# ai-forever/Kandinsky-2

Hardware: NVIDIA H100
Metric: unet_denoising_steps_per_sec (higher is better)
Workload: dtype f16

## Files before the change

kandinsky-2_b200/csrc/k2_api.cu:

```cuda
#include <stdio.h>
#include <stdlib.h>
#include <string.h>

#include <algorithm>
#include <atomic>
#include <mutex>

#include "../../include/k2b200.h"
#include "k2_internal.h"

namespace k2 {

static thread_local std::string g_err;
static std::atomic<long long> g_launches{0};
static int g_force_bn = 0;
static int g_force_split = 0;
static int g_pdl = 0;


void set_error(const std::string& msg) { g_err = msg; }
int fail(const std::string& msg) {
  g_err = msg;
  return -1;
}
void count_launch(int n) { g_launches.fetch_add(n, std::memory_order_relaxed); }

bool pdl_enabled() { return g_pdl != 0; }
static int g_conv_epi_sets = 1;
static int g_gn_bps = 0;
int gn_apply_blocks_per_sm() { return g_gn_bps; }
static int g_attn_half = 1;
// ... 90 lines not shown
    }
  }
  const int k = (!single_image_only && best_tiles[1] * 100 <= best_tiles[0] * 85) ? 1 : 0;
  TN = bn[k];
  TW = bw[k];
  TH = bh[k];
}


struct ConvPlan {
  int TN, TH, TW, tiles_w, tiles_h, tiles_n, m_tiles;
  int m_tiles_phase;
  int BN, splits;
  int fuse_stats, row_groups;
  int es;
};

static void plan_conv(int NB, int H, int W, bool any9, int kchunks, int Cout, int out_mode, bool has_workspace,
                      long long workspace_bytes, bool want_gn, ConvPlan& pl, const int* cfg = nullptr, bool up2 = false,
                      bool w_batched = false) {
  const int g_force_bn = (cfg && cfg[0]) ? cfg[0] : k2::g_force_bn;
  const int g_force_split = (cfg && cfg[2]) ? cfg[2] : k2::g_force_split;
  pl.es = (cfg && cfg[3]) ? cfg[3] : k2::g_conv_epi_sets;
  choose_tile(NB, H, W, pl.TN, pl.TH, pl.TW, w_batched);
  pl.tiles_w = (W + pl.TW - 1) / pl.TW;
  pl.tiles_h = (H + pl.TH - 1) / pl.TH;
  pl.tiles_n = (NB + pl.TN - 1) / pl.TN;
  pl.m_tiles = pl.tiles_w * pl.tiles_h * pl.tiles_n;
  pl.m_tiles_phase = pl.m_tiles;

// ... 34 lines not shown
        if (g_force_split > 0 && sp != g_force_split) continue;
        if (!split_ok(sp)) continue;
        const long long c = model(bn, sp);
        if (best < 0 || c < best) {
          best = c;
          best_bn = bn;
          best_sp = sp;
        }
      }
    }
    BN = best_bn;
    splits = best_sp;
  }
  pl.BN = BN;
  pl.splits = splits;

  pl.fuse_stats = 0;
  pl.row_groups = 0;
  if (want_gn && out_mode == 0 && Cout % 8 == 0) {
    if (splits == 1 && BN >= 64 && Cout % 64 == 0 && (pl.TN == 1 || pl.TH * pl.TW == 16)) {
      pl.fuse_stats = 1;
      pl.row_groups = ((pl.TN == 1) ? pl.m_tiles : NB * pl.tiles_h * pl.tiles_w) * (up2 ? 4 : 1);
    } else if (splits > 1 && (static_cast<long long>(H) * W) % 16 == 0) {
      pl.fuse_stats = 2;
      pl.row_groups = static_cast<int>(M_total / 16);
    }
  }
}

static void plan_to_info(const ConvPlan& pl, int* info) {
  if (!info) return;
  info[0] = pl.BN; info[1] = 0;
  info[2] = pl.splits; info[3] = pl.m_tiles; info[4] = pl.TN;
  info[5] = pl.fuse_stats; info[6] = pl.row_groups;
}

}

using namespace k2;

extern "C" {

const char* k2_last_error(void) { return g_err.c_str(); }
int k2_version(void) { return 100; }
long long k2_launch_count(void) { return g_launches.load(); }
void k2_reset_launch_count(void) { g_launches.store(0); }
int k2_set_tuning(int key, int value) {
  if (key == 0) {
    g_force_bn = value;
    return 0;
  }
  if (key == 1) {
    g_force_split = value;
    return 0;
  }
  if (key == 2) {
    if (value == 2) return fail("k2_set_tuning: no CTA-pair conv kernel on sm_90");
    return 0;
  }
  if (key == 4) {
    g_pdl = value;
    return 0;
  }
  if (key == 10) {
    g_conv_epi_sets = (value == 2) ? 2 : 1;
    return 0;
  }
  if (key == 11) {
    g_gn_bps = value;
    return 0;
  }
  if (key == 9) {
// ... 11 lines not shown
  return k2_conv_gemm_cfg(srcs, nsrc, NB, H, W, w_packed, w_rows, Ktot, ldw, Cout, bias, residual, ldr, out, ldo, out_mode,
                          workspace, workspace_bytes, gn_partial, info, nullptr, 0, stream);
}

int k2_conv_gemm_cfg(const K2ConvSrc* srcs, int nsrc, int NB, int H, int W, const void* w_packed, int w_rows,
                     int Ktot, int ldw, int Cout, const float* bias, const void* residual, int ldr, void* out, int ldo,
                     int out_mode, void* workspace, long long workspace_bytes, float* gn_partial, int* info,
                     const int* cfg, long long w_batch_stride, k2_stream_t stream) {
  K2_REQUIRE(w_batch_stride >= 0 && w_batch_stride % 8 == 0, "conv_gemm_cfg: w_batch_stride must be a multiple of 8 elements");
  const bool w_batched = w_batch_stride > 0;
  if (cfg) {
    K2_REQUIRE(cfg[0] == 0 || cfg[0] == 16 || cfg[0] == 64 || cfg[0] == 128 || cfg[0] == 192 || cfg[0] == 256,
               "conv_gemm_cfg: N tile must be 0, 16, 64, 128, 192 or 256");
    K2_REQUIRE(cfg[1] >= 0 && cfg[1] <= 2 && cfg[2] >= 0 && cfg[2] <= 8 && cfg[3] >= 0 && cfg[3] <= 2,
               "conv_gemm_cfg: pair mode in 0..2, splits in 0..8, epilogue sets in 0..2");
    K2_REQUIRE(cfg[1] != 2, "conv_gemm_cfg: no CTA-pair conv kernel on sm_90");
  }
  K2_REQUIRE(nsrc >= 1 && nsrc <= 3, "conv_gemm: 1..3 sources");
  K2_REQUIRE(NB > 0 && H > 0 && W > 0 && Cout > 0, "conv_gemm: bad geometry");
  K2_REQUIRE(w_rows >= Cout, "conv_gemm: w_rows < Cout");
  K2_REQUIRE(Ktot % 64 == 0, "conv_gemm: Ktot must be a multiple of 64");
  if (ldw == 0) ldw = Ktot;
  K2_REQUIRE(ldw >= Ktot && ldw % 8 == 0 && (reinterpret_cast<uintptr_t>(w_packed) & 15) == 0,
             "conv_gemm: weight row stride / alignment");
  ConvGemmParams p;
  memset(&p, 0, sizeof p);
  p.NB = NB;
  p.H = H;
  p.W = W;
  bool any9 = false;
  int kchunks = 0;
// ... 13 lines not shown
    K2_REQUIRE(src.C > 0 && src.C % 8 == 0 && src.ld % 8 == 0 && src.ld >= src.C, "conv_gemm: bad source C/ld");
    K2_REQUIRE((reinterpret_cast<uintptr_t>(src.ptr) & 15) == 0, "conv_gemm: source not 16B aligned");
    any9 = any9 || src.taps == 9;
    p.seg_taps[s] = src.taps;
    p.seg_kchunks[s] = (src.C + 63) / 64;
    kchunks += src.taps * p.seg_kchunks[s];
  }
  K2_REQUIRE(kchunks * 64 * (up2 ? 4 : 1) == Ktot,
             "conv_gemm: Ktot does not match the sources (taps * ceil(C/64)*64 summed; x4 phases for a taps == 4 source)");
  p.num_k_chunks = kchunks;

  ConvPlan pl;
  plan_conv(NB, H, W, any9 || up2, kchunks, Cout, out_mode, workspace != nullptr, workspace_bytes, gn_partial != nullptr, pl,
            cfg, up2, w_batched);
  K2_REQUIRE(!w_batched || (!up2 && pl.TN == 1), "conv_gemm_cfg: batched weights need single-image tiles");
  p.w_batched = w_batched ? 1 : 0;
  plan_to_info(pl, info);
  p.TN = pl.TN;
  p.TH = pl.TH;
  p.TW = pl.TW;
  p.tiles_w = pl.tiles_w;
  p.tiles_h = pl.tiles_h;
  p.tiles_n = pl.tiles_n;
  p.m_tiles = up2 ? 4 * pl.m_tiles_phase : pl.m_tiles;
  p.m_tiles_phase = pl.m_tiles_phase;
  p.up2 = up2 ? 1 : 0;
  p.a_box_bytes = static_cast<uint32_t>(p.TN * p.TH * p.TW * 128);
  for (int s = 0; s < nsrc; ++s) {
    const K2ConvSrc& src = srcs[s];
    uint64_t dims[4] = {static_cast<uint64_t>(src.C), static_cast<uint64_t>(W), static_cast<uint64_t>(H),
// ... 2 lines not shown
                       static_cast<uint64_t>(src.ld) * 2 * W * H};
    uint32_t box[4] = {64, static_cast<uint32_t>(p.TW), static_cast<uint32_t>(p.TH), static_cast<uint32_t>(p.TN)};
    if (encode_tmap_f16(&p.tmA[s], src.ptr, 4, dims, str, box)) return -1;
  }
  const int BN = pl.BN, splits = pl.splits, fuse_stats = pl.fuse_stats;
  p.splits = splits;
  p.k_per_split = (kchunks + splits - 1) / splits;
  p.M_total = static_cast<long long>(NB) * H * W * (up2 ? 4 : 1);
  p.ws = reinterpret_cast<float*>(workspace);
  p.n_tiles = (Cout + BN - 1) / BN;
  p.Cout = Cout;
  {
    uint64_t dims[3] = {static_cast<uint64_t>(Ktot), static_cast<uint64_t>(w_rows), static_cast<uint64_t>(w_batched ? NB : 1)};
    uint64_t str[2] = {static_cast<uint64_t>(ldw) * 2,
                       (w_batched ? static_cast<uint64_t>(w_batch_stride) : static_cast<uint64_t>(ldw) * w_rows) * 2};
    uint32_t box[3] = {64, static_cast<uint32_t>(BN), 1};
    if (encode_tmap_f16(&p.tmB, w_packed, 3, dims, str, box)) return -1;
  }
  p.bias = bias;
  p.residual = reinterpret_cast<const __half*>(residual);
  p.ldr = ldr;
  p.out = out;
  p.ldo = ldo;
  p.out_mode = (splits > 1) ? 2 : out_mode;
  p.gn_part = (fuse_stats == 1) ? reinterpret_cast<float2*>(gn_partial) : nullptr;
  p.gn_mode = (fuse_stats == 1) ? (p.TN == 1 ? 1 : 2) : 0;
  if (out_mode == 0) {
    K2_REQUIRE(ldo % 8 == 0 && (reinterpret_cast<uintptr_t>(out) & 15) == 0, "conv_gemm: out alignment");
    if (residual)
      K2_REQUIRE(ldr % 8 == 0 && (reinterpret_cast<uintptr_t>(residual) & 15) == 0, "conv_gemm: residual alignment");
  }
  int rc = launch_conv_gemm(p, BN, pl.es, static_cast<cudaStream_t>(stream));
  if (rc == 0) g_launches.fetch_add(1, std::memory_order_relaxed);
  if (rc == 0 && splits > 1) {
    rc = launch_splitk_finalize(p.ws, splits, p.M_total, Cout, bias, p.residual, ldr, reinterpret_cast<__half*>(out), ldo,
                                fuse_stats == 2 ? reinterpret_cast<float2*>(gn_partial) : nullptr,
                                static_cast<cudaStream_t>(stream));
    if (rc == 0) g_launches.fetch_add(1, std::memory_order_relaxed);
  }
  return rc;
}

int k2_conv_plan(int NB, int H, int W, int taps, int Ktot, int Cout, int out_mode, long long workspace_bytes,
                 int want_gn_partial, int* info) {
  K2_REQUIRE(NB > 0 && H > 0 && W > 0 && Cout > 0 && info, "conv_plan: bad arguments");
  K2_REQUIRE(Ktot > 0 && Ktot % 64 == 0, "conv_plan: Ktot must be a positive multiple of 64");
  ConvPlan pl;
// ... 7 lines not shown
```

kandinsky-2_b200/csrc/k2_common.cuh:

```cuda
#pragma once
#include <cuda.h>
#include <cuda_fp16.h>
#include <cuda_runtime.h>
#include <stdint.h>
#include <stdio.h>

namespace k2 {

__device__ __forceinline__ uint32_t smem_u32(const void* p) {
  return static_cast<uint32_t>(__cvta_generic_to_shared(p));
}

__device__ __forceinline__ uint32_t lane_id() { return threadIdx.x & 31; }

__device__ __forceinline__ bool elect_one() {
  uint32_t pred = 0;
  asm volatile(
      "{\n"
      ".reg .b32 rx;\n"
      ".reg .pred px;\n"
      "elect.sync rx|px, 0xffffffff;\n"
      "selp.b32 %0, 1, 0, px;\n"
      "}\n"
      : "=r"(pred));
// ... 1 lines not shown
}

__device__ __forceinline__ void mbar_init(uint64_t* bar, uint32_t count) {
  asm volatile("mbarrier.init.shared::cta.b64 [%0], %1;" ::"r"(smem_u32(bar)), "r"(count));
}
__device__ __forceinline__ void fence_barrier_init() {
  asm volatile("fence.mbarrier_init.release.cluster;" ::: "memory");
}
__device__ __forceinline__ void mbar_arrive_expect_tx(uint64_t* bar, uint32_t bytes) {
  asm volatile("mbarrier.arrive.expect_tx.shared::cta.b64 _, [%0], %1;" ::"r"(smem_u32(bar)),
               "r"(bytes)
               : "memory");
}
__device__ __forceinline__ void mbar_arrive(uint64_t* bar) {
  asm volatile("mbarrier.arrive.shared::cta.b64 _, [%0];" ::"r"(smem_u32(bar)) : "memory");
}
__device__ __forceinline__ bool mbar_try_wait(uint64_t* bar, uint32_t parity) {
  uint32_t ok;
  asm volatile(
      "{\n"
      ".reg .pred p;\n"
      "mbarrier.try_wait.parity.shared::cta.b64 p, [%1], %2;\n"
      "selp.b32 %0, 1, 0, p;\n"
      "}\n"
      : "=r"(ok)
      : "r"(smem_u32(bar)), "r"(parity)
      : "memory");
  return ok != 0;
}
__device__ __forceinline__ void mbar_wait(uint64_t* bar, uint32_t parity) {
// ... 27 lines not shown
                                            int c1) {
  asm volatile(
      "cp.async.bulk.tensor.2d.shared::cluster.global.mbarrier::complete_tx::bytes [%0], [%1, {%3, "
      "%4}], [%2];"
      ::"r"(smem_u32(dst)),
      "l"(reinterpret_cast<uint64_t>(tm)), "r"(smem_u32(bar)), "r"(c0), "r"(c1)
      : "memory");
}
__device__ __forceinline__ void tma_load_3d(void* dst, const CUtensorMap* tm, uint64_t* bar, int c0,
                                            int c1, int c2) {
  asm volatile(
      "cp.async.bulk.tensor.3d.shared::cluster.global.mbarrier::complete_tx::bytes [%0], [%1, {%3, "
      "%4, %5}], [%2];"
      ::"r"(smem_u32(dst)),
      "l"(reinterpret_cast<uint64_t>(tm)), "r"(smem_u32(bar)), "r"(c0), "r"(c1), "r"(c2)
      : "memory");
}
__device__ __forceinline__ void tma_load_4d(void* dst, const CUtensorMap* tm, uint64_t* bar, int c0,
                                            int c1, int c2, int c3) {
  asm volatile(
      "cp.async.bulk.tensor.4d.shared::cluster.global.mbarrier::complete_tx::bytes [%0], [%1, {%3, "
      "%4, %5, %6}], [%2];"
      ::"r"(smem_u32(dst)),
      "l"(reinterpret_cast<uint64_t>(tm)), "r"(smem_u32(bar)), "r"(c0), "r"(c1), "r"(c2), "r"(c3)
      : "memory");
}

__device__ __forceinline__ uint64_t make_wgmma_desc(uint32_t smem_addr) {
  uint64_t d = 0;
  d |= static_cast<uint64_t>((smem_addr & 0x3FFFF) >> 4);
// ... 159 lines not shown
```

kandinsky-2_b200/csrc/k2_conv_gemm.cu:

```cuda
#include <stdio.h>

#include "k2_common.cuh"
#include "k2_internal.h"

namespace k2 {

namespace {

constexpr int BM = 128;
constexpr int BK = 64;
constexpr int A_STAGE_BYTES = BM * BK * 2;
constexpr int ACC_PAD = 4;

constexpr int EPI_STAGE_FLOATS = 32 * 33;
constexpr int EPI_BYTES = 4 * EPI_STAGE_FLOATS * 4 + 4 * 256 * 4;
constexpr int SMEM_LIMIT = 227 * 1024;

template <int BN, int ES>
struct Cfg {
  static constexpr int B_STAGE_BYTES = BN * BK * 2;
  static constexpr int STAGE_BYTES = A_STAGE_BYTES + B_STAGE_BYTES;
  static constexpr int BNC = (BN < 64) ? BN : (ES == 2 ? 128 : 64);
  static_assert(ES == 1 || BN % 128 == 0, "two epilogue sets need N tiles of 128 or 256");
  static constexpr int ACC_BYTES = BM * (BNC + ACC_PAD) * 4;
  static constexpr int BAR_BYTES = 256;
  static constexpr int FIXED = ACC_BYTES + ES * EPI_BYTES + BAR_BYTES + 1024;
  static constexpr int STAGES = (SMEM_LIMIT - FIXED) / STAGE_BYTES > 6 ? 6 : (SMEM_LIMIT - FIXED) / STAGE_BYTES;
  static constexpr int SMEM_BYTES = STAGES * STAGE_BYTES + FIXED;
  static_assert(STAGES >= 2, "conv_gemm: shared memory does not hold two pipeline stages");
};

__device__ __forceinline__ void decode_m_tile(const ConvGemmParams& p, int m_idx, int& n0, int& y0,
                                              int& x0, int& phase) {
  phase = 0;
  if (p.up2) {
    phase = m_idx / p.m_tiles_phase;
    m_idx -= phase * p.m_tiles_phase;
  }
  int tw_i = m_idx % p.tiles_w;
  int t = m_idx / p.tiles_w;
  int th_i = t % p.tiles_h;
  int tn_i = t / p.tiles_h;
  x0 = tw_i * p.TW;
  y0 = th_i * p.TH;
  n0 = tn_i * p.TN;
}

template <int N>
__device__ __forceinline__ void acc_ld(const float* src, uint32_t (&r)[N]) {
#pragma unroll
  for (int v = 0; v < N / 4; ++v) {
    const float4 t = *reinterpret_cast<const float4*>(src + 4 * v);
    r[4 * v] = __float_as_uint(t.x);
    r[4 * v + 1] = __float_as_uint(t.y);
    r[4 * v + 2] = __float_as_uint(t.z);
// ... 283 lines not shown
__global__ void __launch_bounds__(384, 1) conv_gemm_kernel(const __grid_constant__ ConvGemmParams p) {
  using C = Cfg<BN, ES>;
  constexpr int BNC = C::BNC;
  constexpr int NA = BN / 2;
  extern __shared__ uint8_t smem_raw[];
  uint8_t* smem = reinterpret_cast<uint8_t*>((reinterpret_cast<uintptr_t>(smem_raw) + 1023) &
                                             ~static_cast<uintptr_t>(1023));
  float* acc_smem = reinterpret_cast<float*>(smem + C::STAGES * C::STAGE_BYTES);
  float* stat_smem = reinterpret_cast<float*>(smem + C::STAGES * C::STAGE_BYTES + C::ACC_BYTES);
  uint64_t* full_bar = reinterpret_cast<uint64_t*>(smem + C::STAGES * C::STAGE_BYTES + C::ACC_BYTES + ES * EPI_BYTES);
  uint64_t* empty_bar = full_bar + C::STAGES;

  const int warp_idx = threadIdx.x >> 5;
  const int lane = threadIdx.x & 31;
  const int wg = warp_idx >> 2;

  if (threadIdx.x == 0) {
    tma_prefetch_desc(&p.tmB);
    for (int s = 0; s < 3; ++s)
      if (p.seg_taps[s]) tma_prefetch_desc(&p.tmA[s]);
    for (int i = 0; i < C::STAGES; ++i) {
      mbar_init(&full_bar[i], 1);
      mbar_init(&empty_bar[i], 8);
    }
    fence_barrier_init();
  }
  __syncthreads();
  pdl_wait();
  pdl_launch();

  const int total_tiles = p.m_tiles * p.n_tiles * p.splits;

  if (wg == 0) {
    setmaxnreg_dec<40>();
    if (warp_idx == 0 && elect_one()) {
      int stage = 0;
      uint32_t ring_phase = 0;
      const uint32_t tx_bytes = p.a_box_bytes + C::B_STAGE_BYTES;
      for (int tile = blockIdx.x; tile < total_tiles; tile += gridDim.x) {
        const int m_idx = tile % p.m_tiles;
        const int n_idx = (tile / p.m_tiles) % p.n_tiles;
        const int split = tile / (p.m_tiles * p.n_tiles);
        int n0, y0, x0, phase;
        decode_m_tile(p, m_idx, n0, y0, x0, phase);
        const int kb = phase * p.num_k_chunks;
        const int k0 = split * p.k_per_split;
        const int k1 = min(p.num_k_chunks, k0 + p.k_per_split);
        int s = 0, rem = k0;
        while (rem >= p.seg_taps[s] * p.seg_kchunks[s]) {
          rem -= p.seg_taps[s] * p.seg_kchunks[s];
          ++s;
        }
        int tap = rem / p.seg_kchunks[s];
        int c = rem - tap * p.seg_kchunks[s];
        for (int kc = k0; kc < k1; ++kc) {
          const int taps = p.seg_taps[s];
          const int dy = (taps == 9) ? (tap / 3 - 1) : (taps == 4 ? (tap >> 1) + (phase >> 1) - 1 : 0);
          const int dx = (taps == 9) ? (tap % 3 - 1) : (taps == 4 ? (tap & 1) + (phase & 1) - 1 : 0);
          mbar_wait_lean(&empty_bar[stage], ring_phase ^ 1);
          uint8_t* sA = smem + stage * C::STAGE_BYTES;
          uint8_t* sB = sA + A_STAGE_BYTES;
          mbar_arrive_expect_tx(&full_bar[stage], tx_bytes);
          tma_load_4d(sA, &p.tmA[s], &full_bar[stage], c * BK, x0 + dx, y0 + dy, n0);
          tma_load_3d(sB, &p.tmB, &full_bar[stage], (kb + kc) * BK, n_idx * BN, p.w_batched ? n0 : 0);
          if (++stage == C::STAGES) {
            stage = 0;
            ring_phase ^= 1;
          }
          if (++c == p.seg_kchunks[s]) {
            c = 0;
            if (++tap == taps) {
              tap = 0;
              ++s;
            }
          }
        }
      }
    }
  } else {
    setmaxnreg_inc<232>();
    const int g = wg - 1;
    const int w = warp_idx & 3;
    int stage = 0;
    uint32_t phase = 0;
    for (int tile = blockIdx.x; tile < total_tiles; tile += gridDim.x) {
      const int m_idx = tile % p.m_tiles;
      const int n_idx = (tile / p.m_tiles) % p.n_tiles;
      const int split = tile / (p.m_tiles * p.n_tiles);
      const int nk = min(p.num_k_chunks, (split + 1) * p.k_per_split) - split * p.k_per_split;
      float acc[NA];
#pragma unroll
      for (int i = 0; i < NA; ++i) acc[i] = 0.f;
      int prev_stage = -1;
      for (int kc = 0; kc < nk; ++kc) {
        mbar_wait_lean(&full_bar[stage], phase);
        const uint32_t a_addr = smem_u32(smem + stage * C::STAGE_BYTES) + g * (64 * 128);
        const uint32_t b_addr = smem_u32(smem + stage * C::STAGE_BYTES + A_STAGE_BYTES);
        wgmma_fence();
#pragma unroll
        for (int k = 0; k < BK / 16; ++k) {
          const uint64_t adesc = make_wgmma_desc(a_addr) + static_cast<uint64_t>(k * 2);
          const uint64_t bdesc = make_wgmma_desc(b_addr) + static_cast<uint64_t>(k * 2);
          if constexpr (BN == 256) {
            wgmma_m64n256k16(acc, adesc, bdesc, 1u);
          } else if constexpr (BN == 192) {
            wgmma_m64n192k16(acc, adesc, bdesc, 1u);
          } else if constexpr (BN == 128) {
            wgmma_m64n128k16(acc, adesc, bdesc, 1u);
          } else if constexpr (BN == 64) {
            wgmma_m64n64k16(acc, adesc, bdesc, 1u);
          } else {
            static_assert(BN == 16, "conv_gemm: N tile without a wgmma shape");
            wgmma_m64n16k16(acc, adesc, bdesc, 1u);
          }
        }
        wgmma_commit();
        wgmma_wait<1>();
        if (prev_stage >= 0 && lane == 0) mbar_arrive(&empty_bar[prev_stage]);
        prev_stage = stage;
        if (++stage == C::STAGES) {
          stage = 0;
          phase ^= 1;
        }
      }
      wgmma_wait<0>();
      if (prev_stage >= 0 && lane == 0) mbar_arrive(&empty_bar[prev_stage]);

      int n0, y0, x0, mphase;
      decode_m_tile(p, m_idx, n0, y0, x0, mphase);
      const int r0 = 64 * g + 16 * w + (lane >> 2);
      const int cq = 2 * (lane & 3);
#pragma unroll
      for (int pass = 0; pass < BN / BNC; ++pass) {
        named_bar_sync(3, 256);
#pragma unroll
        for (int i = 0; i < NA; i += 2) {
          if ((8 * (i >> 2)) / BNC != pass) continue;
          const int row = r0 + 8 * ((i >> 1) & 1);
          const int col = 8 * (i >> 2) - pass * BNC + cq;
          *reinterpret_cast<float2*>(acc_smem + row * (BNC + ACC_PAD) + col) = make_float2(acc[i], acc[i + 1]);
        }
        named_bar_sync(3, 256);
        if (ES == 2 || g == 0)
          epilogue_tile<BNC, ES>(p, acc_smem, w, lane, n0, y0, x0, n_idx * BN + pass * BNC, split, m_idx, stat_smem, g,
                                 mphase);
      }
    }
  }
}

__global__ void __launch_bounds__(256) splitk_finalize_kernel(const float* __restrict__ ws, int splits, long long M,
                                                              int Cout, const float* __restrict__ bias,
                                                              const __half* __restrict__ residual, int ldr,
                                                              __half* __restrict__ out, int ldo, float2* __restrict__ gn_part) {
  __shared__ float red[8][32][17];
  const int vx = threadIdx.x & 31, ry = threadIdx.x >> 5;
  const int c0 = (blockIdx.y * 32 + vx) * 8;
  const long long rg = blockIdx.x;
  pdl_wait();
  pdl_launch();
  float st[16];
#pragma unroll
  for (int e = 0; e < 16; ++e) st[e] = 0.f;
// ... 44 lines not shown
  const int vx2 = threadIdx.x >> 3, e2 = threadIdx.x & 7;
  const int c = (blockIdx.y * 32 + vx2) * 8 + e2;
  if (c < Cout) {
    float s1 = 0.f, s2 = 0.f;
#pragma unroll
    for (int q = 0; q < 8; ++q) {
      s1 += red[q][vx2][e2];
      s2 += red[q][vx2][8 + e2];
    }
    gn_part[rg * Cout + c] = make_float2(s1, s2);
  }
}


template <int BN, int ES>
int launch_bn(const ConvGemmParams& p, cudaStream_t stream) {
  using C = Cfg<BN, ES>;
  static bool attr_set = false;
  if (!attr_set) {
    K2_CHECK_CUDA(cudaFuncSetAttribute(conv_gemm_kernel<BN, ES>, cudaFuncAttributeMaxDynamicSharedMemorySize,
                                       C::SMEM_BYTES));
    attr_set = true;
  }
  int total = p.m_tiles * p.n_tiles * p.splits;
  int grid = total < num_sms() ? total : num_sms();
  K2_CHECK_CUDA(launch_k(conv_gemm_kernel<BN, ES>, dim3(grid), dim3(384), C::SMEM_BYTES, stream, p));
  return 0;
}

}

int launch_splitk_finalize(const float* ws, int splits, long long M, int Cout, const float* bias, const __half* residual,
                           int ldr, __half* out, int ldo, float2* gn_part, cudaStream_t stream) {
  dim3 grid(static_cast<unsigned int>((M + 15) / 16), (Cout / 8 + 31) / 32);
  K2_CHECK_CUDA(launch_k(splitk_finalize_kernel, grid, dim3(256), 0, stream, ws, splits, M, Cout, bias, residual, ldr, out, ldo,
                         gn_part));
  return 0;
}

int launch_conv_gemm(const ConvGemmParams& p, int BN, int epilogue_sets, cudaStream_t stream) {
  if (epilogue_sets == 2) {
    switch (BN) {
      case 128: return launch_bn<128, 2>(p, stream);
      case 256: return launch_bn<256, 2>(p, stream);
      default: break;
    }
  }
  switch (BN) {
    case 16: return launch_bn<16, 1>(p, stream);
    case 64: return launch_bn<64, 1>(p, stream);
    case 128: return launch_bn<128, 1>(p, stream);
    case 192: return launch_bn<192, 1>(p, stream);
    case 256: return launch_bn<256, 1>(p, stream);
    default: return fail("conv_gemm: unsupported BN");
  }
}

}
```

kandinsky-2_b200/csrc/k2_internal.h:

```cpp
#pragma once
#include <cuda.h>
#include <cuda_fp16.h>
#include <cuda_runtime.h>
#include <stdint.h>

#include <string>

namespace k2 {

void set_error(const std::string& msg);
int fail(const std::string& msg);
#define K2_CHECK_CUDA(expr)                                                                 \
  do {                                                                                      \
    cudaError_t _e = (expr);                                                                \
    if (_e != cudaSuccess)                                                                  \
      return ::k2::fail(std::string(#expr) + ": " + cudaGetErrorString(_e));                \
  } while (0)
#define K2_REQUIRE(cond, msg)                                  \
  do {                                                         \
    if (!(cond)) return ::k2::fail(std::string("k2b200: ") + (msg)); \
  } while (0)

int num_sms();
bool pdl_enabled();

template <typename... KArgs, typename... Args>
inline cudaError_t launch_k(void (*kernel)(KArgs...), dim3 grid, dim3 block, size_t smem, cudaStream_t stream,
                            Args&&... args) {
  cudaLaunchConfig_t cfg = {};
  cfg.gridDim = grid;
  cfg.blockDim = block;
  cfg.dynamicSmemBytes = smem;
  cfg.stream = stream;
  cudaLaunchAttribute attr[1];
  attr[0].id = cudaLaunchAttributeProgrammaticStreamSerialization;
  attr[0].val.programmaticStreamSerializationAllowed = 1;
  cfg.attrs = attr;
  cfg.numAttrs = pdl_enabled() ? 1 : 0;
  return cudaLaunchKernelEx(&cfg, kernel, static_cast<KArgs>(args)...);
}
void count_launch(int n = 1);

int encode_tmap_f16(CUtensorMap* out, const void* base, int rank, const uint64_t* dims,
                    const uint64_t* strides_bytes , const uint32_t* box);

struct ConvGemmParams {
  CUtensorMap tmA[3];
  CUtensorMap tmB;
  int w_batched;
  int seg_taps[3];
  int seg_kchunks[3];
  int num_k_chunks;
  int NB, H, W;
  int TN, TH, TW;
// ... 4 lines not shown
  const __half* residual;
  int ldr;
  void* out;
  int ldo;
  int out_mode;
  uint32_t a_box_bytes;
  int splits;
  int k_per_split;
  float* ws;
  long long M_total;
  float2* gn_part;
  int gn_mode;
  int up2;
  int m_tiles_phase;
};
int launch_conv_gemm(const ConvGemmParams& p, int BN, int epilogue_sets, cudaStream_t stream);
int launch_splitk_finalize(const float* ws, int splits, long long M, int Cout, const float* bias, const __half* residual,
                           int ldr, __half* out, int ldo, float2* gn_part, cudaStream_t stream);

struct FlashParams {
  const __half* qkv;
  long long ldq;
  int hs, q_off, k_off, v_off;
  const __half* enc;
  long long lde;
  int ehs, ek_off, ev_off;
  int B, heads, T, Tc;
  __half* out;
  int ldo, ohs;
  float scale_log2e;
};
// ... 6 lines not shown
```

kandinsky-2_b200/kandinsky2/launch_plan.py:

```python
import os

import torch

from . import ops

FOLD_MAX_RG = int(os.environ.get("K2_GN_FOLD_MAX_RG", "18"))
TUNE = os.environ.get("K2_AUTOTUNE", "1") != "0"
FORK = os.environ.get("K2_FORK", "1") != "0"
TUNE_SMALL_M = int(os.environ.get("K2_TUNE_SMALL_M", "8192"))
_tune_cache = {}


def tune(key, run, m_rows=0):
    if not TUNE:
        return None
    key = (torch.cuda.current_device(), TUNE_SMALL_M) + key
    if key in _tune_cache:
        return _tune_cache[key]
    info = [0] * 7
    run(None, info)
    bn0, splits = info[0], info[2]
    cout = key[3]
    best = None
    if cout > 64:
        bns = [bn0] if splits > 1 else [bn for bn in (128, 192, 256) if bn - 64 < cout or bn == bn0]
        cands = [(bn0, 0, splits, 1)] + [(bn, 0, splits, es) for bn in bns for es in ((1,) if bn == 192 else (1, 2))
                                        if (bn, es) != (bn0, 1)]
        if 0 < m_rows <= TUNE_SMALL_M and splits == 1:
            for bn in (128, 192, 256):
                if bn - 64 >= cout:
                    continue
                for sp in (2, 3, 4):
                    probe = [0] * 7
                    try:
                        run((bn, 1, sp, 1), probe)
                    except Exception:
                        continue
                    if probe[0] == bn and probe[2] == sp:
                        cands.append((bn, 1, sp, 1))

        def timed(cfg, reps=6):
            run(cfg)
            evs = [torch.cuda.Event(enable_timing=True) for _ in range(reps + 1)]
            evs[0].record()
            for i in range(reps):
                run(cfg)
                evs[i + 1].record()
            torch.cuda.synchronize()
            return min(evs[i].elapsed_time(evs[i + 1]) for i in range(reps))

        t0 = tb = timed(cands[0])
        for cfg in cands[1:]:
            t = timed(cfg)
            if t < tb and t < 0.97 * t0:
                t = max(t, timed(cfg))
                if t < tb and t < 0.97 * t0:
                    best, tb = cfg, t
    _tune_cache[key] = best
    return best


class LaunchPlan:
    def __init__(self, dev, nb):
        self.dev = dev
        self.NB = nb
        self._parts = {}
        self._scratch = {}
        self.steps = []
        self.graph = None
        self._side_stream = None
        self._side_open = False
        self._serial = False
# ... 149 lines not shown
```

profiles/conv_layers.py:

```python
import argparse
import json
import os
import subprocess
import sys

ROOT = os.path.dirname(os.path.dirname(os.path.abspath(__file__)))
for p in (ROOT, os.path.join(ROOT, "kandinsky-2_b200")):
    if p not in sys.path:
        sys.path.insert(0, p)

import torch

B, H, W = 4, 96, 96


def _card():
    q = subprocess.run(["nvidia-smi", "--query-gpu=name,power.limit,clocks.max.sm", "--format=csv,noheader", "-i", "0"],
                       capture_output=True, text=True)
    return q.stdout.strip() or torch.cuda.get_device_name(0)


def _pad64(c):
    return (c + 63) // 64 * 64

# ... 51 lines not shown
    reps = max(10, int(min_ms / max(s.elapsed_time(e) / 5, 1e-3)) + 1)
    s.record()
    for _ in range(reps):
        run(cfg)
    e.record()
    torch.cuda.synchronize()
    return s.elapsed_time(e) / reps, reps


def main():
    ap = argparse.ArgumentParser()
    ap.add_argument("--out", default=None)
    ap.add_argument("--min-ms", type=float, default=50.0, help="timed window per configuration")
    ap.add_argument("--mma-n", default="tile", choices=["tile", "64"],
                    help="wgmma N of the build: one instruction per N tile, or m64n64k16 per 64 columns")
    args = ap.parse_args()
    if not torch.cuda.is_available():
        raise SystemExit("needs a CUDA sm_90 device")
    import bench
    from kandinsky2 import launch_plan, ops
    from kandinsky2.model.gaussian_diffusion import FusedStep, create_ddpm_v22
    dev = torch.device("cuda", 0)
    torch.cuda.set_device(dev)
    ops.set_tuning(4, 1)
    res = {"card": _card(), "torch": torch.__version__, "geometry": f"cfg-2: UNet batch {2 * B}, {H}x{W} latents",
           "mma_n": args.mma_n, "min_ms": args.min_ms}

    counts = {}
    tune = launch_plan.tune

    def counting_tune(key, run, m_rows=0):
        counts[key] = counts.get(key, 0) + 1
        return tune(key, run, m_rows=m_rows)
    launch_plan.tune = counting_tune
    model = bench.build_unet(dev)
    image_emb = torch.randn(2 * B, 1280, generator=torch.Generator().manual_seed(1234)).to(dev)
    step = FusedStep(model, B, H, W, dict(image_emb=image_emb), guidance_scale=4.0, cond_first=False, clip_range=2.0,
                     threshold_mode=0)
    launch_plan.tune = tune
    diffusion = create_ddpm_v22(50)
    coef, ts = diffusion._tables(dev)
# ... 3 lines not shown
    x.copy_(torch.randn(B, 4, H, W, device=dev))
    step.advance(x)
    torch.cuda.synchronize()
    res["plan_conv_launches"] = sum(1 for _, kind, _ in step.plan.steps if kind == "conv_gemm")
    res["counted_conv_launches"] = sum(counts.values())

    g = torch.Generator(device=dev).manual_seed(7)
    layers = []
    for key, n in counts.items():
        run, shp = _layer(key, dev, g)
        if run is None:
            continue
        info = [0] * 7
        picked = launch_plan._tune_cache.get((dev.index, launch_plan.TUNE_SMALL_M) + key)
        run(picked, info)
        picked_cfg = [info[0], 0, info[2], (picked[3] if picked and picked[3] else 1)]
        cout = shp["N"]
        cfgs = []
        if cout > 64:
            cfgs = [(bn, 0, 1, es) for bn in (128, 192, 256) if bn - 64 < cout or bn == info[0]
                    for es in ((1,) if bn == 192 else (1, 2))]
        if tuple(picked_cfg) not in cfgs:
            cfgs.append(tuple(picked_cfg))
        rows = []
        for cfg in cfgs:
            info = [0] * 7
            run(cfg, info)
            bn, splits = info[0], info[2]
            ms, reps = _time(run, cfg, args.min_ms)
            flops = 2.0 * shp["M"] * cout * shp["K"]
            mma_n = bn if (args.mma_n == "tile" or bn < 64) else 64
            smem_bpf = (2048 + 32 * mma_n) / (2.0 * 64 * mma_n * 16)
            m_tiles = info[3] * (4 if "up2" in shp["desc"] else 1)
            chunks = m_tiles * ((cout + bn - 1) // bn) * (shp["K"] // 64)
            l2_bytes = chunks * (16384 + bn * 128)
            rows.append(dict(n_tile=bn, epilogue_sets=cfg[3], splits=splits, ms=round(ms, 5), reps=reps,
                             tflops=round(flops / (ms * 1e-3) / 1e12, 1),
                             smem_operand_bytes_per_flop=round(smem_bpf, 5),
                             l2_operand_bytes_per_flop=round(l2_bytes / flops, 5),
                             l2_operand_TBps=round(l2_bytes / (ms * 1e-3) / 1e12, 2)))
        pick = next((r for r in rows if [r["n_tile"], r["splits"], r["epilogue_sets"]] ==
                     [picked_cfg[0], picked_cfg[2], picked_cfg[3]]), rows[0])
        layers.append(dict(shape=shp["desc"], key=repr(key), launches_per_step=n, gemm_gflop=round(2e-9 * shp["M"] * cout * shp["K"], 3),
                           picked=dict(n_tile=picked_cfg[0], splits=picked_cfg[2], epilogue_sets=picked_cfg[3],
                                       tuned=picked is not None),
                           picked_ms=pick["ms"], configs=rows))
    total = sum(l["launches_per_step"] * l["picked_ms"] for l in layers)
    for l in layers:
        l["share_of_conv_time"] = round(l["launches_per_step"] * l["picked_ms"] / total, 4)
    layers.sort(key=lambda l: -l["share_of_conv_time"])
    res["conv_ms_per_step_at_picked"] = round(total, 3)
    res["layers"] = layers

    print(f"# {res['card']}  (mma_n={args.mma_n})  conv time per step at the picked configurations: {total:.2f} ms")
    print(f"{'shape':44s} {'n':>2s} {'share':>6s} {'pick':>9s}  " + "  ".join(f"{c:>9s}" for c in
          ("128/1", "128/2", "192/1", "256/1", "256/2")) + "   (TFLOP/s at N tile / epilogue sets, splits 1)")
    for l in layers:
        by = {(r["n_tile"], r["epilogue_sets"]): r["tflops"] for r in l["configs"] if r["splits"] == 1}
        pk = l["picked"]
        print(f"{l['shape'][:44]:44s} {l['launches_per_step']:2d} {100 * l['share_of_conv_time']:5.1f}% "
              f"{pk['n_tile']:>3d}/{pk['epilogue_sets']}/{pk['splits']:<3d}  " +
              "  ".join(f"{by.get(c, float('nan')):9.1f}" for c in ((128, 1), (128, 2), (192, 1), (256, 1), (256, 2))))
    if args.out:
        os.makedirs(os.path.dirname(os.path.abspath(args.out)), exist_ok=True)
        with open(args.out, "w") as f:
            f.write(json.dumps(res, indent=1) + "\n")


if __name__ == "__main__":
    main()
```

Baseline: 27.45.

## Add 2-CTA cluster mode multicasting conv weight tiles via TMA

Adds a CTA-pair (cluster of 2) path to the implicit-GEMM conv kernel. Each CTA loads half of the weight tile and multicasts it to both CTAs, and the empty barriers are released across the cluster. The goal is to halve L2 traffic for weight operands. The autotuner now also times pair configurations for BN=256 and uses a revised incumbent-comparison loop, so pairs run only where they measure faster. This costs cluster synchronization, phantom tiles when the M tile count is odd, and cross-CTA barrier coupling.

```diff
diff --git a/kandinsky-2_b200/csrc/k2_api.cu b/kandinsky-2_b200/csrc/k2_api.cu
--- a/kandinsky-2_b200/csrc/k2_api.cu
+++ b/kandinsky-2_b200/csrc/k2_api.cu
@@ -15,6 +15,7 @@
 static std::atomic<long long> g_launches{0};
 static int g_force_bn = 0;
 static int g_force_split = 0;
+static int g_cta_pair = 0;
 static int g_pdl = 0;
 
 
@@ -135,6 +136,7 @@
   int BN, splits;
   int fuse_stats, row_groups;
   int es;
+  int pair;
 };
 
 static void plan_conv(int NB, int H, int W, bool any9, int kchunks, int Cout, int out_mode, bool has_workspace,
@@ -199,6 +201,8 @@
   }
   pl.BN = BN;
   pl.splits = splits;
+  const int pair = (cfg && cfg[1]) ? cfg[1] : k2::g_cta_pair;
+  pl.pair = (pair == 2 && BN >= 128 && !w_batched) ? 1 : 0;
 
   pl.fuse_stats = 0;
   pl.row_groups = 0;
@@ -215,7 +219,7 @@
 
 static void plan_to_info(const ConvPlan& pl, int* info) {
   if (!info) return;
-  info[0] = pl.BN; info[1] = 0;
+  info[0] = pl.BN; info[1] = pl.pair ? 2 : 0;
   info[2] = pl.splits; info[3] = pl.m_tiles; info[4] = pl.TN;
   info[5] = pl.fuse_stats; info[6] = pl.row_groups;
 }
@@ -240,7 +244,8 @@
     return 0;
   }
   if (key == 2) {
-    if (value == 2) return fail("k2_set_tuning: no CTA-pair conv kernel on sm_90");
+    if (value < 0 || value > 2) return fail("k2_set_tuning: CTA-pair mode must be 0, 1 or 2");
+    g_cta_pair = value;
     return 0;
   }
   if (key == 4) {
@@ -282,7 +287,6 @@
                "conv_gemm_cfg: N tile must be 0, 16, 64, 128, 192 or 256");
     K2_REQUIRE(cfg[1] >= 0 && cfg[1] <= 2 && cfg[2] >= 0 && cfg[2] <= 8 && cfg[3] >= 0 && cfg[3] <= 2,
                "conv_gemm_cfg: pair mode in 0..2, splits in 0..8, epilogue sets in 0..2");
-    K2_REQUIRE(cfg[1] != 2, "conv_gemm_cfg: no CTA-pair conv kernel on sm_90");
   }
   K2_REQUIRE(nsrc >= 1 && nsrc <= 3, "conv_gemm: 1..3 sources");
   K2_REQUIRE(NB > 0 && H > 0 && W > 0 && Cout > 0, "conv_gemm: bad geometry");
@@ -326,6 +330,9 @@
   plan_conv(NB, H, W, any9 || up2, kchunks, Cout, out_mode, workspace != nullptr, workspace_bytes, gn_partial != nullptr, pl,
             cfg, up2, w_batched);
   K2_REQUIRE(!w_batched || (!up2 && pl.TN == 1), "conv_gemm_cfg: batched weights need single-image tiles");
+  K2_REQUIRE(!(cfg && cfg[1] == 2) || pl.pair,
+             w_batched ? "conv_gemm_cfg: CTA pairs share one weight tile; per-image weights (w_batch_stride > 0) run single-CTA"
+                       : "conv_gemm_cfg: CTA pairs need N tile 128, 192 or 256 (the weight tile is split in two 1024-byte-aligned halves)");
   p.w_batched = w_batched ? 1 : 0;
   plan_to_info(pl, info);
   p.TN = pl.TN;
@@ -358,7 +365,7 @@
     uint64_t dims[3] = {static_cast<uint64_t>(Ktot), static_cast<uint64_t>(w_rows), static_cast<uint64_t>(w_batched ? NB : 1)};
     uint64_t str[2] = {static_cast<uint64_t>(ldw) * 2,
                        (w_batched ? static_cast<uint64_t>(w_batch_stride) : static_cast<uint64_t>(ldw) * w_rows) * 2};
-    uint32_t box[3] = {64, static_cast<uint32_t>(BN), 1};
+    uint32_t box[3] = {64, static_cast<uint32_t>(pl.pair ? BN / 2 : BN), 1};
     if (encode_tmap_f16(&p.tmB, w_packed, 3, dims, str, box)) return -1;
   }
   p.bias = bias;
@@ -374,7 +381,7 @@
     if (residual)
       K2_REQUIRE(ldr % 8 == 0 && (reinterpret_cast<uintptr_t>(residual) & 15) == 0, "conv_gemm: residual alignment");
   }
-  int rc = launch_conv_gemm(p, BN, pl.es, static_cast<cudaStream_t>(stream));
+  int rc = launch_conv_gemm(p, BN, pl.es, pl.pair != 0, static_cast<cudaStream_t>(stream));
   if (rc == 0) g_launches.fetch_add(1, std::memory_order_relaxed);
   if (rc == 0 && splits > 1) {
     rc = launch_splitk_finalize(p.ws, splits, p.M_total, Cout, bias, p.residual, ldr, reinterpret_cast<__half*>(out), ldo,
diff --git a/kandinsky-2_b200/csrc/k2_common.cuh b/kandinsky-2_b200/csrc/k2_common.cuh
--- a/kandinsky-2_b200/csrc/k2_common.cuh
+++ b/kandinsky-2_b200/csrc/k2_common.cuh
@@ -39,6 +39,30 @@
 }
 __device__ __forceinline__ void mbar_arrive(uint64_t* bar) {
   asm volatile("mbarrier.arrive.shared::cta.b64 _, [%0];" ::"r"(smem_u32(bar)) : "memory");
+}
+__device__ __forceinline__ void mbar_arrive_cluster(uint64_t* bar, uint32_t cta_rank) {
+  asm volatile(
+      "{\n"
+      ".reg .b32 ra;\n"
+      "mapa.shared::cluster.u32 ra, %0, %1;\n"
+      "mbarrier.arrive.shared::cluster.b64 _, [ra];\n"
+      "}\n" ::"r"(smem_u32(bar)),
+      "r"(cta_rank)
+      : "memory");
+}
+
+__device__ __forceinline__ uint32_t cluster_nctarank() {
+  uint32_t r;
+  asm volatile("mov.u32 %0, %%cluster_nctarank;" : "=r"(r));
+  return r;
+}
+__device__ __forceinline__ uint32_t cluster_ctarank() {
+  uint32_t r;
+  asm volatile("mov.u32 %0, %%cluster_ctarank;" : "=r"(r));
+  return r;
+}
+__device__ __forceinline__ void cluster_sync() {
+  asm volatile("barrier.cluster.arrive.release;\nbarrier.cluster.wait.acquire;" ::: "memory");
 }
 __device__ __forceinline__ bool mbar_try_wait(uint64_t* bar, uint32_t parity) {
   uint32_t ok;
@@ -96,6 +120,15 @@
       "%4, %5}], [%2];"
       ::"r"(smem_u32(dst)),
       "l"(reinterpret_cast<uint64_t>(tm)), "r"(smem_u32(bar)), "r"(c0), "r"(c1), "r"(c2)
+      : "memory");
+}
+__device__ __forceinline__ void tma_load_3d_multicast(void* dst, const CUtensorMap* tm, uint64_t* bar, int c0, int c1, int c2,
+                                                      uint16_t cta_mask) {
+  asm volatile(
+      "cp.async.bulk.tensor.3d.shared::cluster.global.mbarrier::complete_tx::bytes.multicast::cluster [%0], [%1, {%3, "
+      "%4, %5}], [%2], %6;"
+      ::"r"(smem_u32(dst)),
+      "l"(reinterpret_cast<uint64_t>(tm)), "r"(smem_u32(bar)), "r"(c0), "r"(c1), "r"(c2), "h"(cta_mask)
       : "memory");
 }
 __device__ __forceinline__ void tma_load_4d(void* dst, const CUtensorMap* tm, uint64_t* bar, int c0,
diff --git a/kandinsky-2_b200/csrc/k2_conv_gemm.cu b/kandinsky-2_b200/csrc/k2_conv_gemm.cu
--- a/kandinsky-2_b200/csrc/k2_conv_gemm.cu
+++ b/kandinsky-2_b200/csrc/k2_conv_gemm.cu
@@ -30,15 +30,28 @@
   static_assert(STAGES >= 2, "conv_gemm: shared memory does not hold two pipeline stages");
 };
 
-__device__ __forceinline__ void decode_m_tile(const ConvGemmParams& p, int m_idx, int& n0, int& y0,
-                                              int& x0, int& phase) {
-  phase = 0;
-  if (p.up2) {
-    phase = m_idx / p.m_tiles_phase;
-    m_idx -= phase * p.m_tiles_phase;
-  }
-  int tw_i = m_idx % p.tiles_w;
-  int t = m_idx / p.tiles_w;
+struct Tile {
+  int m_idx, n_idx, split, phase, box;
+  bool phantom;
+};
+__device__ __forceinline__ int m_groups_phase(const ConvGemmParams& p, int cs) { return (p.m_tiles_phase + cs - 1) / cs; }
+__device__ __forceinline__ Tile tile_of(const ConvGemmParams& p, int q, int cs, int rank) {
+  const int gpp = m_groups_phase(p, cs);
+  const int m_groups = gpp * (p.up2 ? 4 : 1);
+  Tile t;
+  const int gi = q % m_groups;
+  t.n_idx = (q / m_groups) % p.n_tiles;
+  t.split = q / (m_groups * p.n_tiles);
+  t.phase = gi / gpp;
+  t.box = (gi - t.phase * gpp) * cs + rank;
+  t.phantom = t.box >= p.m_tiles_phase;
+  t.m_idx = t.phase * p.m_tiles_phase + t.box;
+  return t;
+}
+
+__device__ __forceinline__ void decode_box(const ConvGemmParams& p, int box, int& n0, int& y0, int& x0) {
+  int tw_i = box % p.tiles_w;
+  int t = box / p.tiles_w;
   int th_i = t % p.tiles_h;
   int tn_i = t / p.tiles_h;
   x0 = tw_i * p.TW;
@@ -352,6 +365,8 @@
   const int warp_idx = threadIdx.x >> 5;
   const int lane = threadIdx.x & 31;
   const int wg = warp_idx >> 2;
+  const int cs = static_cast<int>(cluster_nctarank());
+  const int rank = static_cast<int>(cluster_ctarank());
 
   if (threadIdx.x == 0) {
     tma_prefetch_desc(&p.tmB);
@@ -359,28 +374,35 @@
       if (p.seg_taps[s]) tma_prefetch_desc(&p.tmA[s]);
     for (int i = 0; i < C::STAGES; ++i) {
       mbar_init(&full_bar[i], 1);
-      mbar_init(&empty_bar[i], 8);
+      mbar_init(&empty_bar[i], 8 * cs);
     }
     fence_barrier_init();
   }
-  __syncthreads();
+  if (cs == 2)
+    cluster_sync();
+  else
+    __syncthreads();
   pdl_wait();
   pdl_launch();
 
-  const int total_tiles = p.m_tiles * p.n_tiles * p.splits;
+  const int total_units = m_groups_phase(p, cs) * (p.up2 ? 4 : 1) * p.n_tiles * p.splits;
+  const int unit0 = blockIdx.x / cs, units_step = gridDim.x / cs;
 
   if (wg == 0) {
     setmaxnreg_dec<40>();
     if (warp_idx == 0 && elect_one()) {
       int stage = 0;
       uint32_t ring_phase = 0;
-      const uint32_t tx_bytes = p.a_box_bytes + C::B_STAGE_BYTES;
-      for (int tile = blockIdx.x; tile < total_tiles; tile += gridDim.x) {
-        const int m_idx = tile % p.m_tiles;
-        const int n_idx = (tile / p.m_tiles) % p.n_tiles;
-        const int split = tile / (p.m_tiles * p.n_tiles);
-        int n0, y0, x0, phase;
-        decode_m_tile(p, m_idx, n0, y0, x0, phase);
+      constexpr int B_HALF = C::B_STAGE_BYTES / 2;
+      for (int q = unit0; q < total_units; q += units_step) {
+        const Tile t = tile_of(p, q, cs, rank);
+        const int n_idx = t.n_idx, split = t.split, phase = t.phase;
+        int n0, y0, x0;
+        decode_box(p, t.box, n0, y0, x0);
+        const uint32_t tx_bytes = (t.phantom ? 0u : p.a_box_bytes) + C::B_STAGE_BYTES;
+        int b_row = n_idx * BN + rank * (BN / 2);
+        if (cs == 1 || b_row >= p.Cout) b_row = n_idx * BN;
+        const int b_off = (cs == 1) ? 0 : rank * B_HALF;
         const int kb = phase * p.num_k_chunks;
         const int k0 = split * p.k_per_split;
         const int k1 = min(p.num_k_chunks, k0 + p.k_per_split);
@@ -397,10 +419,13 @@
           const int dx = (taps == 9) ? (tap % 3 - 1) : (taps == 4 ? (tap & 1) + (phase & 1) - 1 : 0);
           mbar_wait_lean(&empty_bar[stage], ring_phase ^ 1);
           uint8_t* sA = smem + stage * C::STAGE_BYTES;
-          uint8_t* sB = sA + A_STAGE_BYTES;
+          uint8_t* sB = sA + A_STAGE_BYTES + b_off;
           mbar_arrive_expect_tx(&full_bar[stage], tx_bytes);
-          tma_load_4d(sA, &p.tmA[s], &full_bar[stage], c * BK, x0 + dx, y0 + dy, n0);
-          tma_load_3d(sB, &p.tmB, &full_bar[stage], (kb + kc) * BK, n_idx * BN, p.w_batched ? n0 : 0);
+          if (!t.phantom) tma_load_4d(sA, &p.tmA[s], &full_bar[stage], c * BK, x0 + dx, y0 + dy, n0);
+          if (cs == 1)
+            tma_load_3d(sB, &p.tmB, &full_bar[stage], (kb + kc) * BK, b_row, p.w_batched ? n0 : 0);
+          else
+            tma_load_3d_multicast(sB, &p.tmB, &full_bar[stage], (kb + kc) * BK, b_row, 0, 0x3);
           if (++stage == C::STAGES) {
             stage = 0;
             ring_phase ^= 1;
@@ -421,10 +446,13 @@
     const int w = warp_idx & 3;
     int stage = 0;
     uint32_t phase = 0;
-    for (int tile = blockIdx.x; tile < total_tiles; tile += gridDim.x) {
-      const int m_idx = tile % p.m_tiles;
-      const int n_idx = (tile / p.m_tiles) % p.n_tiles;
-      const int split = tile / (p.m_tiles * p.n_tiles);
+    auto release = [&](int s) {
+      mbar_arrive(&empty_bar[s]);
+      if (cs == 2) mbar_arrive_cluster(&empty_bar[s], rank ^ 1);
+    };
+    for (int q = unit0; q < total_units; q += units_step) {
+      const Tile t = tile_of(p, q, cs, rank);
+      const int m_idx = t.m_idx, n_idx = t.n_idx, split = t.split;
       const int nk = min(p.num_k_chunks, (split + 1) * p.k_per_split) - split * p.k_per_split;
       float acc[NA];
 #pragma unroll
@@ -454,7 +482,7 @@
         }
         wgmma_commit();
         wgmma_wait<1>();
-        if (prev_stage >= 0 && lane == 0) mbar_arrive(&empty_bar[prev_stage]);
+        if (prev_stage >= 0 && lane == 0) release(prev_stage);
         prev_stage = stage;
         if (++stage == C::STAGES) {
           stage = 0;
@@ -462,10 +490,12 @@
         }
       }
       wgmma_wait<0>();
-      if (prev_stage >= 0 && lane == 0) mbar_arrive(&empty_bar[prev_stage]);
-
-      int n0, y0, x0, mphase;
-      decode_m_tile(p, m_idx, n0, y0, x0, mphase);
+      if (prev_stage >= 0 && lane == 0) release(prev_stage);
+      if (t.phantom) continue;
+
+      const int mphase = t.phase;
+      int n0, y0, x0;
+      decode_box(p, t.box, n0, y0, x0);
       const int r0 = 64 * g + 16 * w + (lane >> 2);
       const int cq = 2 * (lane & 3);
 #pragma unroll
@@ -485,6 +515,7 @@
       }
     }
   }
+  if (cs == 2) cluster_sync();
 }
 
 __global__ void __launch_bounds__(256) splitk_finalize_kernel(const float* __restrict__ ws, int splits, long long M,
@@ -559,17 +590,34 @@
 
 
 template <int BN, int ES>
-int launch_bn(const ConvGemmParams& p, cudaStream_t stream) {
+int launch_bn(const ConvGemmParams& p, int cs, cudaStream_t stream) {
   using C = Cfg<BN, ES>;
   static bool attr_set = false;
+  static int max_pairs = 0;
   if (!attr_set) {
     K2_CHECK_CUDA(cudaFuncSetAttribute(conv_gemm_kernel<BN, ES>, cudaFuncAttributeMaxDynamicSharedMemorySize,
                                        C::SMEM_BYTES));
     attr_set = true;
   }
-  int total = p.m_tiles * p.n_tiles * p.splits;
-  int grid = total < num_sms() ? total : num_sms();
-  K2_CHECK_CUDA(launch_k(conv_gemm_kernel<BN, ES>, dim3(grid), dim3(384), C::SMEM_BYTES, stream, p));
+  if (cs == 2 && max_pairs == 0) {
+    cudaLaunchConfig_t lc = {};
+    lc.gridDim = dim3(2 * num_sms());
+    lc.blockDim = dim3(384);
+    lc.dynamicSmemBytes = C::SMEM_BYTES;
+    cudaLaunchAttribute attr[1];
+    attr[0].id = cudaLaunchAttributeClusterDimension;
+    attr[0].val.clusterDim.x = 2;
+    attr[0].val.clusterDim.y = 1;
+    attr[0].val.clusterDim.z = 1;
+    lc.attrs = attr;
+    lc.numAttrs = 1;
+    K2_CHECK_CUDA(cudaOccupancyMaxActiveClusters(&max_pairs, conv_gemm_kernel<BN, ES>, &lc));
+    if (max_pairs <= 0) return fail("conv_gemm: no 2-CTA cluster of this kernel fits on the device");
+  }
+  const int units = (p.m_tiles_phase + cs - 1) / cs * (p.up2 ? 4 : 1) * p.n_tiles * p.splits;
+  const int slots = (cs == 2) ? max_pairs : num_sms();
+  const int grid = (units < slots ? units : slots) * cs;
+  K2_CHECK_CUDA(launch_k_cluster(conv_gemm_kernel<BN, ES>, dim3(grid), dim3(384), C::SMEM_BYTES, stream, cs, p));
   return 0;
 }
 
@@ -583,20 +631,22 @@
   return 0;
 }
 
-int launch_conv_gemm(const ConvGemmParams& p, int BN, int epilogue_sets, cudaStream_t stream) {
+int launch_conv_gemm(const ConvGemmParams& p, int BN, int epilogue_sets, bool cta_pair, cudaStream_t stream) {
+  if (cta_pair && (BN < 128 || p.w_batched)) return fail("conv_gemm: CTA pairs need N tile 128, 192 or 256 and one weight matrix");
+  const int cs = cta_pair ? 2 : 1;
   if (epilogue_sets == 2) {
     switch (BN) {
-      case 128: return launch_bn<128, 2>(p, stream);
-      case 256: return launch_bn<256, 2>(p, stream);
+      case 128: return launch_bn<128, 2>(p, cs, stream);
+      case 256: return launch_bn<256, 2>(p, cs, stream);
       default: break;
     }
   }
   switch (BN) {
-    case 16: return launch_bn<16, 1>(p, stream);
-    case 64: return launch_bn<64, 1>(p, stream);
-    case 128: return launch_bn<128, 1>(p, stream);
-    case 192: return launch_bn<192, 1>(p, stream);
-    case 256: return launch_bn<256, 1>(p, stream);
+    case 16: return launch_bn<16, 1>(p, cs, stream);
+    case 64: return launch_bn<64, 1>(p, cs, stream);
+    case 128: return launch_bn<128, 1>(p, cs, stream);
+    case 192: return launch_bn<192, 1>(p, cs, stream);
+    case 256: return launch_bn<256, 1>(p, cs, stream);
     default: return fail("conv_gemm: unsupported BN");
   }
 }
diff --git a/kandinsky-2_b200/csrc/k2_internal.h b/kandinsky-2_b200/csrc/k2_internal.h
--- a/kandinsky-2_b200/csrc/k2_internal.h
+++ b/kandinsky-2_b200/csrc/k2_internal.h
@@ -25,19 +25,35 @@
 bool pdl_enabled();
 
 template <typename... KArgs, typename... Args>
-inline cudaError_t launch_k(void (*kernel)(KArgs...), dim3 grid, dim3 block, size_t smem, cudaStream_t stream,
-                            Args&&... args) {
+inline cudaError_t launch_k_cluster(void (*kernel)(KArgs...), dim3 grid, dim3 block, size_t smem, cudaStream_t stream,
+                                    int cluster_x, Args&&... args) {
   cudaLaunchConfig_t cfg = {};
   cfg.gridDim = grid;
   cfg.blockDim = block;
   cfg.dynamicSmemBytes = smem;
   cfg.stream = stream;
-  cudaLaunchAttribute attr[1];
-  attr[0].id = cudaLaunchAttributeProgrammaticStreamSerialization;
-  attr[0].val.programmaticStreamSerializationAllowed = 1;
+  cudaLaunchAttribute attr[2];
+  int n = 0;
+  if (pdl_enabled()) {
+    attr[n].id = cudaLaunchAttributeProgrammaticStreamSerialization;
+    attr[n].val.programmaticStreamSerializationAllowed = 1;
+    ++n;
+  }
+  if (cluster_x > 1) {
+    attr[n].id = cudaLaunchAttributeClusterDimension;
+    attr[n].val.clusterDim.x = static_cast<unsigned int>(cluster_x);
+    attr[n].val.clusterDim.y = 1;
+    attr[n].val.clusterDim.z = 1;
+    ++n;
+  }
   cfg.attrs = attr;
-  cfg.numAttrs = pdl_enabled() ? 1 : 0;
+  cfg.numAttrs = n;
   return cudaLaunchKernelEx(&cfg, kernel, static_cast<KArgs>(args)...);
+}
+template <typename... KArgs, typename... Args>
+inline cudaError_t launch_k(void (*kernel)(KArgs...), dim3 grid, dim3 block, size_t smem, cudaStream_t stream,
+                            Args&&... args) {
+  return launch_k_cluster(kernel, grid, block, smem, stream, 1, static_cast<Args&&>(args)...);
 }
 void count_launch(int n = 1);
 
@@ -72,7 +88,7 @@
   int up2;
   int m_tiles_phase;
 };
-int launch_conv_gemm(const ConvGemmParams& p, int BN, int epilogue_sets, cudaStream_t stream);
+int launch_conv_gemm(const ConvGemmParams& p, int BN, int epilogue_sets, bool cta_pair, cudaStream_t stream);
 int launch_splitk_finalize(const float* ws, int splits, long long M, int Cout, const float* bias, const __half* residual,
                            int ldr, __half* out, int ldo, float2* gn_part, cudaStream_t stream);
 
diff --git a/kandinsky-2_b200/kandinsky2/launch_plan.py b/kandinsky-2_b200/kandinsky2/launch_plan.py
--- a/kandinsky-2_b200/kandinsky2/launch_plan.py
+++ b/kandinsky-2_b200/kandinsky2/launch_plan.py
@@ -38,6 +38,18 @@
                         continue
                     if probe[0] == bn and probe[2] == sp:
                         cands.append((bn, 1, sp, 1))
+        pairs = []
+        for bn, _, sp, es in cands:
+            if bn != 256 or (bn, 2, sp, es) in pairs:
+                continue
+            probe = [0] * 7
+            try:
+                run((bn, 2, sp, es), probe)
+            except Exception:
+                continue
+            if probe[1] == 2:
+                pairs.append((bn, 2, sp, es))
+        cands += pairs
 
         def timed(cfg, reps=6):
             run(cfg)
@@ -49,13 +61,13 @@
             torch.cuda.synchronize()
             return min(evs[i].elapsed_time(evs[i + 1]) for i in range(reps))
 
-        t0 = tb = timed(cands[0])
+        inc = cands[0]
         for cfg in cands[1:]:
-            t = timed(cfg)
-            if t < tb and t < 0.97 * t0:
-                t = max(t, timed(cfg))
-                if t < tb and t < 0.97 * t0:
-                    best, tb = cfg, t
+            for _ in range(2):
+                if timed(cfg) >= 0.97 * timed(inc):
+                    break
+            else:
+                best = inc = cfg
     _tune_cache[key] = best
     return best
 
diff --git a/profiles/conv_layers.py b/profiles/conv_layers.py
--- a/profiles/conv_layers.py
+++ b/profiles/conv_layers.py
@@ -89,6 +89,7 @@
     ap.add_argument("--min-ms", type=float, default=50.0, help="timed window per configuration")
     ap.add_argument("--mma-n", default="tile", choices=["tile", "64"],
                     help="wgmma N of the build: one instruction per N tile, or m64n64k16 per 64 columns")
+    ap.add_argument("--no-pairs", action="store_true", help="time single-CTA configurations only (a build without pair mode)")
     args = ap.parse_args()
     if not torch.cuda.is_available():
         raise SystemExit("needs a CUDA sm_90 device")
@@ -99,7 +100,7 @@
     torch.cuda.set_device(dev)
     ops.set_tuning(4, 1)
     res = {"card": _card(), "torch": torch.__version__, "geometry": f"cfg-2: UNet batch {2 * B}, {H}x{W} latents",
-           "mma_n": args.mma_n, "min_ms": args.min_ms}
+           "mma_n": args.mma_n, "pairs": not args.no_pairs, "min_ms": args.min_ms}
 
     counts = {}
     tune = launch_plan.tune
@@ -133,12 +134,12 @@
         info = [0] * 7
         picked = launch_plan._tune_cache.get((dev.index, launch_plan.TUNE_SMALL_M) + key)
         run(picked, info)
-        picked_cfg = [info[0], 0, info[2], (picked[3] if picked and picked[3] else 1)]
+        picked_cfg = [info[0], info[1], info[2], (picked[3] if picked and picked[3] else 1)]
         cout = shp["N"]
         cfgs = []
         if cout > 64:
-            cfgs = [(bn, 0, 1, es) for bn in (128, 192, 256) if bn - 64 < cout or bn == info[0]
-                    for es in ((1,) if bn == 192 else (1, 2))]
+            cfgs = [(bn, cp, 1, es) for bn in (128, 192, 256) if bn - 64 < cout or bn == info[0]
+                    for es in ((1,) if bn == 192 else (1, 2)) for cp in ((0,) if args.no_pairs else (0, 2))]
         if tuple(picked_cfg) not in cfgs:
             cfgs.append(tuple(picked_cfg))
         rows = []
@@ -152,17 +153,16 @@
             smem_bpf = (2048 + 32 * mma_n) / (2.0 * 64 * mma_n * 16)
             m_tiles = info[3] * (4 if "up2" in shp["desc"] else 1)
             chunks = m_tiles * ((cout + bn - 1) // bn) * (shp["K"] // 64)
-            l2_bytes = chunks * (16384 + bn * 128)
-            rows.append(dict(n_tile=bn, epilogue_sets=cfg[3], splits=splits, ms=round(ms, 5), reps=reps,
+            l2_bytes = chunks * (16384 + bn * 128 // (2 if info[1] == 2 else 1))
+            rows.append(dict(n_tile=bn, epilogue_sets=cfg[3], cta_pair=info[1], splits=splits, ms=round(ms, 5), reps=reps,
                              tflops=round(flops / (ms * 1e-3) / 1e12, 1),
                              smem_operand_bytes_per_flop=round(smem_bpf, 5),
                              l2_operand_bytes_per_flop=round(l2_bytes / flops, 5),
                              l2_operand_TBps=round(l2_bytes / (ms * 1e-3) / 1e12, 2)))
-        pick = next((r for r in rows if [r["n_tile"], r["splits"], r["epilogue_sets"]] ==
-                     [picked_cfg[0], picked_cfg[2], picked_cfg[3]]), rows[0])
+        pick = next((r for r in rows if [r["n_tile"], r["cta_pair"], r["splits"], r["epilogue_sets"]] == picked_cfg), rows[0])
         layers.append(dict(shape=shp["desc"], key=repr(key), launches_per_step=n, gemm_gflop=round(2e-9 * shp["M"] * cout * shp["K"], 3),
-                           picked=dict(n_tile=picked_cfg[0], splits=picked_cfg[2], epilogue_sets=picked_cfg[3],
-                                       tuned=picked is not None),
+                           picked=dict(n_tile=picked_cfg[0], cta_pair=picked_cfg[1], splits=picked_cfg[2],
+                                       epilogue_sets=picked_cfg[3], tuned=picked is not None),
                            picked_ms=pick["ms"], configs=rows))
     total = sum(l["launches_per_step"] * l["picked_ms"] for l in layers)
     for l in layers:
@@ -172,14 +172,16 @@
     res["layers"] = layers
 
     print(f"# {res['card']}  (mma_n={args.mma_n})  conv time per step at the picked configurations: {total:.2f} ms")
-    print(f"{'shape':44s} {'n':>2s} {'share':>6s} {'pick':>9s}  " + "  ".join(f"{c:>9s}" for c in
-          ("128/1", "128/2", "192/1", "256/1", "256/2")) + "   (TFLOP/s at N tile / epilogue sets, splits 1)")
+    cols = [(bn, es, cp) for bn, es in ((128, 1), (128, 2), (192, 1), (256, 1), (256, 2))
+            for cp in ((0,) if args.no_pairs else (0, 2))]
+    print(f"{'shape':44s} {'n':>2s} {'share':>6s} {'pick':>11s}  " + " ".join(f"{f'{bn}/{es}' + ('p' if cp else ''):>7s}"
+          for bn, es, cp in cols) + "   (TFLOP/s at N tile / epilogue sets, p = CTA pair, splits 1)")
     for l in layers:
-        by = {(r["n_tile"], r["epilogue_sets"]): r["tflops"] for r in l["configs"] if r["splits"] == 1}
+        by = {(r["n_tile"], r["epilogue_sets"], r["cta_pair"]): r["tflops"] for r in l["configs"] if r["splits"] == 1}
         pk = l["picked"]
         print(f"{l['shape'][:44]:44s} {l['launches_per_step']:2d} {100 * l['share_of_conv_time']:5.1f}% "
-              f"{pk['n_tile']:>3d}/{pk['epilogue_sets']}/{pk['splits']:<3d}  " +
-              "  ".join(f"{by.get(c, float('nan')):9.1f}" for c in ((128, 1), (128, 2), (192, 1), (256, 1), (256, 2))))
+              f"{pk['n_tile']:>3d}/{pk['epilogue_sets']}/{pk['splits']}{'p' if pk['cta_pair'] == 2 else ' ':<4s}  " +
+              " ".join(f"{by.get(c, float('nan')):7.1f}" for c in cols))
     if args.out:
         os.makedirs(os.path.dirname(os.path.abspath(args.out)), exist_ok=True)
         with open(args.out, "w") as f:
```

After: 27.38, median of 6. Within noise of the previous version (-0.3%).
